# nexus-rl/dfd-starter

Hardware: AMD Instinct MI355X
Metric: env steps/sec (whole node) + sec/FD-grad-step, 4096 antithetic perturbations (higher is better)
Workload: dtype f32; 1 GPU; BASELINE config 3: HalfCheetah-shaped synthetic env (obs 17, act 6), MujocoPolicy(17,6) P=6092, 4096 antithetic perturbations per GPU (2048 directions x +/-), T=1000 fixed-length episodes, full FD step (rollout + weights + gradient + DSGD); perturbations_per_gpu=4096, envs_per_perturbation=1, global_perturbations=4096, episode_len=1000, n_params=6092, parallelism=dp1

## Files before the change

### dfd-starter_amd/csrc/fdr_common.h

```cpp
#pragma once
#include <hip/hip_runtime.h>
#include <stdint.h>

#include "../../include/fdr.h"

namespace fdr {

constexpr int kWave = 64;
constexpr int kHidden = 64;

__host__ __device__ __forceinline__ uint64_t mix64(uint64_t z) {
  z = (z ^ (z >> 30)) * 0xBF58476D1CE4E5B9ull;
  z = (z ^ (z >> 27)) * 0x94D049BB133111EBull;
  return z ^ (z >> 31);
}
__device__ __forceinline__ uint64_t hash_ctr(uint64_t key, uint64_t lane, uint64_t t, uint64_t k) {
  const uint64_t c = (lane << 32) | (t << 4) | k;
  return mix64(key + c * 0x9E3779B97F4A7C15ull);
}
constexpr uint64_t kJiggleT = (1ull << 28) - 1;

__device__ __forceinline__ float uniform24(uint64_t h) {
  return (float)(uint32_t)(h >> 40) * 0x1p-24f;
}
__device__ __forceinline__ float normal_bm(uint64_t h) {
  const float u1 = (float)((uint32_t)(h >> 40) + 1u) * 0x1p-24f;
  const float u2 = (float)((uint32_t)(h >> 16) & 0xFFFFFFu) * 0x1p-24f;
  const float r = __builtin_sqrtf(-1.38629436111989061f * __builtin_amdgcn_logf(u1));
  return r * __builtin_amdgcn_cosf(u2);
}

constexpr float kTanhScale = 2.88539008177792681f;
__device__ __forceinline__ float tanh_pre(float t) {
  const float e = __builtin_amdgcn_exp2f(t);
  return 1.0f - 2.0f * __builtin_amdgcn_rcpf(1.0f + e);
}
__device__ __forceinline__ float tanh_fast(float x) { return tanh_pre(x * kTanhScale); }
template <bool kPre>
__device__ __forceinline__ float tanh_act(float z) {
  if constexpr (kPre) return tanh_pre(z);
  else return tanh_fast(z);
}

__device__ __forceinline__ void wave_lds_sync() {
  __builtin_amdgcn_fence(__ATOMIC_RELEASE, "wavefront");
  __builtin_amdgcn_wave_barrier();
  __builtin_amdgcn_fence(__ATOMIC_ACQUIRE, "wavefront");
}

template <typename T>
__device__ __forceinline__ T wave_sum(T v) {
#pragma unroll
  for (int m = 32; m >= 1; m >>= 1) v += __shfl_xor(v, m, kWave);
  return v;
}

struct ParamSrc {
  const float* base;
  const float* eps;
  float sigma;
  int sgn;
  double n2;

  __device__ __forceinline__ float get(int64_t p) {
#pragma clang fp contract(off)
    const float t = base[p];
    const float st = sigma * eps[p];
    const double d = (double)st;
    n2 += sgn != 0 ? d * d : 0.0;
    return sgn > 0 ? t + st : (sgn < 0 ? t - st : t);
  }
  __device__ __forceinline__ float get_if(int64_t p, bool use) {
#pragma clang fp contract(off)
    const float t = base[p];
    const float st = sigma * eps[p];
    const double d = (double)st;
    n2 += (use && sgn != 0) ? d * d : 0.0;
    return sgn > 0 ? t + st : (sgn < 0 ? t - st : t);
  }
  __device__ __forceinline__ float get_nocount(int64_t p) const {
#pragma clang fp contract(off)
    const float t = base[p];
    const float st = sigma * eps[p];
    return sgn > 0 ? t + st : (sgn < 0 ? t - st : t);
  }
};

}
```

### dfd-starter_amd/csrc/fdr_rollout.hip

```cpp
#include <hip/hip_runtime.h>

#include <cfloat>
#include <cmath>
#include <cstdlib>
#include <cstring>
#include <type_traits>
#include <utility>

#include "fdr_common.h"
#include "fdr_internal.h"
#include "fdr_wave.h"

namespace fdr {

constexpr int kLanesPerBlock = 4;

#ifdef FDR_PHASE_STAMPS
__device__ unsigned long long g_phase_stamps[5];
#endif

__host__ __device__ constexpr int round4(int x) { return (x + 3) / 4 * 4; }

template <int NIN, int NA, bool DISC>
struct Layout {
// ... 636 lines not shown
          mark(2, y);
        } else {
          y = pl.layers23(h1, sc, j, mark, WIDE ? w3reg : nullptr);
        }
        int act_d = 0;
        float act_c = 0.f;
        if constexpr (DISC) {
          float p;
          p = pl.template softmax<kHead2, !kDet>(y, j);
          if constexpr (kHead2 && !kDet) {
    #pragma clang fp contract(off)
            const float tot = p + dpp_mov<kDppQuadXor1>(p);
            const float p0 = dpp_mov<0xA0>(p);
            act_d = p0 <= readlane_f(rbuf, tb) * tot ? 1 : 0;
            eacc -= (j < NA) ? disc_entropy_term(p, tot) : 0.f;
          } else {
          float pv[NA];
    #pragma unroll
          for (int i = 0; i < NA; ++i) pv[i] = readlane_f(p, i);
          float tot = pv[0];
    #pragma unroll
          for (int i = 1; i < NA; ++i) tot += pv[i];
          if constexpr (kDet) {
            float best = pv[0];
    #pragma unroll
            for (int i = 1; i < NA; ++i) {
              act_d = pv[i] > best ? i : act_d;
              best = fmaxf(best, pv[i]);
            }
          } else {
            const float target = readlane_f(rbuf, tb) * tot;
            float c = 0.f;
    #pragma unroll
            for (int i = 0; i < NA - 1; ++i) {
              c += pv[i];
              act_d += c <= target ? 1 : 0;
            }
          }
          eacc -= (j < NA) ? disc_entropy_term(p, tot) : 0.f;
          }
        } else {
          const float th = tanh_fast(y);
          const float sd = std_from_tanh(dpp_mov<kDppRowShl + NA>(th));
          eacc += __builtin_amdgcn_logf(sd);
          act_c = kDet ? th : gauss_action(th, sd, zt);
        }

        mark(3, DISC ? (float)act_d : act_c);
        if constexpr (ENV == FDR_ENV_SYNTH) {
          if constexpr (kCand) {
            s = cand[0];
    #pragma unroll
            for (int i = 1; i < NA; ++i) s = act_d == i ? cand[i] : s;
          } else {
            if constexpr (DISC) {
              pre += mrow[NX + act_d];
            } else {
              float kr[NA];
    #pragma unroll
              for (int m = 0; m < NA; ++m) kr[m] = WIDE ? kreg[m] : mrow[NX + m];
              dpp_tail<NA>(pre, act_c, kr);
            }
            s = tanh_fast(pre);
          }
          racc += (double)s;
          if constexpr (kTerm) {
            if (fabsf(readlane_f(s, a.done_dim)) > a.done_thr) {
              nsteps = t + 1;
              return;
            }
          }
        } else {
          const int prev_x = col * 7;
          const int tc = col + act_d / 3 - 1, tr = row + act_d % 3 - 1;
          if (tc >= 0 && tc < a.map_w && tr >= 0 && tr < a.map_h && a.walkable[tr * a.map_w + tc]) {
            col = tc;
            row = tr;
          }
          racc += (double)(col * 7 - prev_x);
          s = trap_obs(j, col, row);
        }
        mark(4, s);
      }
    }
  };
  if (det)
    episode(std::true_type{});
  else
    episode(std::false_type{});
#ifdef FDR_PHASE_STAMPS
  if (blockIdx.x == 0 && threadIdx.x == 0)
    for (int k = 0; k < 5; ++k) g_phase_stamps[k] = ph_acc[k];
#endif

  eacc *= 0.693147180559945309f;
  const double esum = wave_sum((j < NA) ? (double)eacc : 0.0);
  if (j == 0) {
    double r = racc;
    if (a.jiggle) r += (hash_ctr(key, ulane, kJiggleT, 15) & 1ull) ? 1e-12 : -1e-12;
    a.ret[lane] = r;
    double e = esum / (double)nsteps;
    if constexpr (!DISC) e += (double)NA * 1.4189385332046727;
    a.ent[lane] = e;
    a.steps[lane] = nsteps;
  }
  if constexpr (FEAT & 2) {
    if (j < NIN) {
      a.os_mean[(int64_t)lane * NIN + j] = os_mean;
      a.os_m2[(int64_t)lane * NIN + j] = os_m2;
    }
    if (j == 0) a.os_count[lane] = os_n;
  }
}

constexpr int kPairWaves = 2;

__device__ __forceinline__ f2 tanh2_pre(f2 t) {
  const f2 d = f2{__builtin_amdgcn_exp2f(t.x), __builtin_amdgcn_exp2f(t.y)} + f2{1.f, 1.f};
  return pk_fma(f2{-2.f, -2.f}, f2{__builtin_amdgcn_rcpf(d.x), __builtin_amdgcn_rcpf(d.y)}, f2{1.f, 1.f});
}
__device__ __forceinline__ f2 tanh2_fast(f2 x) {
  return tanh2_pre(x * f2{kTanhScale, kTanhScale});
}
constexpr float kPreScale = kTanhScale;
template <bool kPre>
__device__ __forceinline__ f2 tanh2_act(f2 z) {
  if constexpr (kPre) return tanh2_pre(z);
  else return tanh2_fast(z);
}

template <int NIN, int NA, bool DISC>
struct MlpPair {
  using L = Layout<NIN, NA, DISC>;
  static constexpr int NOUT = L::NOUT;
  static constexpr int NX = round4(NIN);
  static_assert(NX <= 32, "pair kernel: policy input wider than 32");
  static constexpr bool kBiasCol = NIN < NX;
  static constexpr bool kW1Lds = NIN > 8;
  static constexpr bool kPre = !DISC;
  static constexpr float kWS = kPre ? kTanhScale : 1.f;
  static constexpr int kW1Chunks = kW1Lds ? NX / 4 : 0;
  static constexpr int kTileF4 = (2 * kW1Chunks + 8) * kWave;
  f2 w1a[kW1Lds ? 1 : NX / 2], w1b[kW1Lds ? 1 : NX / 2];
  float b1a, b1b;
  const float4* tile;
  f2 w2[64];
  float b2a, b2b, b3;
  float a0, c0, a1a, c1a, a1b, c1b, a2a, c2a, a2b, c2b;

  __host__ __device__ static constexpr int head_unit(int rho, int k, int e) {
    return 32 * rho + 8 * (k >> 2) + 4 * e + (k & 3);
  }

  __device__ __forceinline__ void load(ParamSrc& src, int t, int tid, const float* bn_mean, const float* bn_var,
                                       float4* wave_tile) {
    const int rho = t >> 4, o = t & 15;
    const int ua = 2 * t, ub = 2 * t + 1;
    float4* my = wave_tile + tid;
    tile = my;
    auto w1v = [&](int u, int k) {
      return kWS * (k < NIN ? src.get(L::L1W + (int64_t)u * NIN + k) : (k == NIN ? src.get(L::L1B + u) : 0.f));
    };
    if constexpr (kPk) {
#pragma unroll
      for (int j = 0; j < 2 * kW1Chunks; ++j) {
        const float e0 = w1v(ua, 2 * j), f0 = w1v(ub, 2 * j), e1 = w1v(ua, 2 * j + 1), f1 = w1v(ub, 2 * j + 1);
        my[j * kWave] = float4{e0, f0, e1, f1};
      }
    } else if constexpr (kW1Lds) {
#pragma unroll
      for (int m = 0; m < kW1Chunks; ++m) {
        const float e0 = w1v(ua, 4 * m), e1 = w1v(ua, 4 * m + 1), e2 = w1v(ua, 4 * m + 2), e3 = w1v(ua, 4 * m + 3);
        my[m * kWave] = float4{e0, e1, e2, e3};
        const float f0 = w1v(ub, 4 * m), f1 = w1v(ub, 4 * m + 1), f2_ = w1v(ub, 4 * m + 2), f3 = w1v(ub, 4 * m + 3);
        my[(kW1Chunks + m) * kWave] = float4{f0, f1, f2_, f3};
      }
    } else {
#pragma unroll
      for (int p = 0; p < NX / 2; ++p) {
        const float e0 = w1v(ua, 2 * p), e1 = w1v(ua, 2 * p + 1);
        w1a[p] = f2{e0, e1};
        const float f0 = w1v(ub, 2 * p), f1 = w1v(ub, 2 * p + 1);
        w1b[p] = f2{f0, f1};
      }
    }
    b1a = kBiasCol ? 0.f : kWS * src.get(L::L1B + ua);
    b1b = kBiasCol ? 0.f : kWS * src.get(L::L1B + ub);
    __builtin_amdgcn_sched_barrier(0);
    const int q4 = t >> 2, c4 = t & 3;
#pragma unroll
    for (int p = 0; p < 4; ++p) {
      const int row0 = 8 * q4 + (c4 ^ p), row1 = row0 + 4;
#pragma unroll
      for (int k = 0; k < 16; ++k) {
        const float e0 = src.get(L::L2W + (int64_t)row0 * kHidden + 16 * c4 + k);
        const float e1 = src.get(L::L2W + (int64_t)row1 * kHidden + 16 * c4 + k);
        w2[p * 16 + k] = f2{kWS * e0, kWS * e1};
      }
#pragma unroll
      for (int k = 0; k < 16; ++k) asm volatile("" : "+v"(w2[p * 16 + k]));
      asm volatile("" : "+v"(src.n2));
      __builtin_amdgcn_sched_barrier(0);
    }
    const int u2a = 8 * q4 + c4, u2b = 8 * q4 + 4 + c4;
    b2a = kWS * src.get(L::L2B + u2a);
    b2b = kWS * src.get(L::L2B + u2b);
    {
      const bool has_o = o < NOUT;
      const int oc = has_o ? o : 0;
#pragma unroll
      for (int m = 0; m < 8; ++m) {
        float e[4];
#pragma unroll
        for (int i = 0; i < 4; ++i) {
          const int w = 4 * m + i;
          e[i] = src.get_if(L::L3W + (int64_t)oc * kHidden + head_unit(rho, w & 15, w >> 4), has_o);
        }
        my[(2 * kW1Chunks + m) * kWave] =
            has_o ? float4{kWS * e[0], kWS * e[1], kWS * e[2], kWS * e[3]} : float4{0.f, 0.f, 0.f, 0.f};
      }
      const float b3v = src.get_if(L::L3B + oc, has_o && rho == 0);
      b3 = has_o ? kWS * b3v : 0.f;
    }
    wave_lds_sync();
    a0 = c0 = a1a = c1a = a1b = c1b = a2a = c2a = a2b = c2b = 0.f;
    if constexpr (DISC) {
      const float* bm = bn_mean ? bn_mean : src.base;
      const float* bv = bn_var ? bn_var : src.base;
      auto stat = [&](int k, float& rm, float& rv) {
        const float m = bm[k], v = bv[k];
        rm = bn_mean ? m : 0.f;
        rv = bn_var ? v : 1.f;
      };
      {
        const bool in = t < NIN;
        const int tc = in ? t : 0;
        const float w = src.get_if(L::BN0W + tc, in), b = src.get_if(L::BN0B + tc, in);
        float rm, rv, a, c;
        stat(tc, rm, rv);
        bn_fold(w, b, rm, rv, a, c);
        a0 = in ? a : 0.f;
        c0 = in ? c : 0.f;
      }
      auto fold = [&](int64_t wofs, int64_t bofs, int st, int u, float& av, float& cv) {
        const float w = src.get(wofs + u), b = src.get(bofs + u);
        float rm, rv;
        stat(st + u, rm, rv);
        bn_fold(w, b, rm, rv, av, cv);
      };
      fold(L::BN1W, L::BN1B, NIN, ua, a1a, c1a);
      fold(L::BN1W, L::BN1B, NIN, ub, a1b, c1b);
      fold(L::BN2W, L::BN2B, NIN + kHidden, u2a, a2a, c2a);
      fold(L::BN2W, L::BN2B, NIN + kHidden, u2b, a2b, c2b);
    }
  }

  __device__ __forceinline__ float input_transform(float x) const {
    if constexpr (DISC) {
      return fmaf(x, a0, c0);
    } else {
      return x;
    }
  }

  __device__ __forceinline__ float act1(float z, float av, float cv) const {
    if constexpr (DISC) {
      return fmaf(fmaxf(z, 0.f), av, cv);
    } else {
      return tanh_act<kPre>(z);
    }
  }

  static constexpr bool kTail = kW1Lds && kBiasCol && NX - NIN == 3;
  static constexpr int NQ = kTail ? NX / 4 - 1 : NX / 4;
  static constexpr bool kPk = kW1Lds && kBiasCol;
  static constexpr int kPkPairs = (NIN + 2) / 2;
  struct L1Rows {
    float4 wa[kW1Lds && !kPk ? NQ : 1], wb[kW1Lds && !kPk ? NQ : 1], m[NQ];
    float2 ta, tb;
    float tm;
    float4 wp[kPk ? kPkPairs : 1];
  };
  __device__ __forceinline__ void l1_prefetch(L1Rows& r, const float* mrow) const {
    const float4* m4 = reinterpret_cast<const float4*>(mrow);
#pragma unroll
    for (int q = 0; q < NQ; ++q) {
      if constexpr (kW1Lds && !kPk) {
        r.wa[q] = tile[q * kWave];
        r.wb[q] = tile[(kW1Chunks + q) * kWave];
      }
      r.m[q] = m4[q];
    }
    if constexpr (kPk) {
#pragma unroll
      for (int j = 0; j < kPkPairs; ++j) r.wp[j] = tile[j * kWave];
      if constexpr (kTail) r.tm = mrow[4 * NQ];
    } else if constexpr (kTail) {
      r.ta = *reinterpret_cast<const float2*>(&tile[NQ * kWave]);
      r.tb = *reinterpret_cast<const float2*>(&tile[(kW1Chunks + NQ) * kWave]);
      r.tm = mrow[4 * NQ];
    }
  }

  template <bool kSameInput>
  __device__ __forceinline__ f2 layer1_env(const float* xs, const float* ss, const L1Rows& rows, float& env) const {
    const float4* x4 = reinterpret_cast<const float4*>(xs);
    const float4* s4 = reinterpret_cast<const float4*>(ss);
    return layer1_env_q<kSameInput>([&](int q) { return x4[q]; }, [&](int q) { return s4[q]; }, rows, env,
                                    kTail ? xs[4 * NQ] : 0.f, kTail ? ss[4 * NQ] : 0.f);
  }
  template <bool kSameInput, class XQ, class SQ>
  __device__ __forceinline__ f2 layer1_env_q(XQ&& xq, SQ&& sq, const L1Rows& rows, float& env, float xt,
                                             float st) const {
    f2 aa0 = {b1a, 0.f}, aa1 = {0.f, 0.f}, ab0 = {b1b, 0.f}, ab1 = {0.f, 0.f};
    f2 am0 = {0.f, 0.f}, am1 = {0.f, 0.f};
    if constexpr (kPk) {
      constexpr int NC = 2;
      f2 acc[NC];
#pragma unroll
      for (int q = 0; q < NC; ++q) acc[q] = f2{0.f, 0.f};
#pragma unroll
      for (int q = 0; q < NQ; ++q) {
        const float4 xv = xq(q), mv = rows.m[q];
        const float4 sv = kSameInput ? xv : sq(q);
#pragma unroll
        for (int i = 0; i < 4; ++i) {
          const int k = 4 * q + i;
          if (k < NIN) {
            const float4 w = rows.wp[k >> 1];
            const f2 xp = (i < 2) ? f2{xv.x, xv.y} : f2{xv.z, xv.w};
            if (kPre && k == NIN % NC) {
              const float4 wb = rows.wp[NIN >> 1];
              const f2 bias = (NIN & 1) ? f2{wb.z, wb.w} : f2{wb.x, wb.y};
              acc[k % NC] = (k & 1) ? pk_fma_bhi(f2{w.z, w.w}, xp, bias) : pk_fma_blo(f2{w.x, w.y}, xp, bias);
            } else if (k < NC)
              acc[k % NC] = (k & 1) ? pk_mul_bhi(f2{w.z, w.w}, xp) : pk_mul_blo(f2{w.x, w.y}, xp);
            else
              acc[k % NC] = (k & 1) ? pk_fma_bhi(f2{w.z, w.w}, xp, acc[k % NC]) : pk_fma_blo(f2{w.x, w.y}, xp, acc[k % NC]);
          }
        }
        am0 = pk_fma(f2{mv.x, mv.y}, f2{sv.x, sv.y}, am0);
        am1 = pk_fma(f2{mv.z, mv.w}, f2{sv.z, sv.w}, am1);
      }
      if constexpr (kTail) {
        const float4 w = rows.wp[(NIN - 1) >> 1];
        acc[(NIN - 1) % NC] = pk_fma(((NIN - 1) & 1) ? f2{w.z, w.w} : f2{w.x, w.y}, f2{xt, xt}, acc[(NIN - 1) % NC]);
        am1.x = fmaf(rows.tm, kSameInput ? xt : st, am1.x);
      }
      if constexpr (!kPre || NIN % NC >= NIN) {
        const float4 w = rows.wp[NIN >> 1];
        acc[NIN % NC] = acc[NIN % NC] + ((NIN & 1) ? f2{w.z, w.w} : f2{w.x, w.y});
      }
      const f2 h = acc[0] + acc[1];
      const f2 am = am0 + am1;
      env = am.x + am.y;
      if constexpr (DISC) {
        return f2{act1(h.x, a1a, c1a), act1(h.y, a1b, c1b)};
      } else {
        return tanh2_act<kPre>(h);
      }
    }
#pragma unroll
    for (int q = 0; q < NQ; ++q) {
      const float4 xv = xq(q), mv = rows.m[q];
      const float4 sv = kSameInput ? xv : sq(q);
      float4 wa, wb;
      if constexpr (kW1Lds) {
        wa = rows.wa[q];
        wb = rows.wb[q];
      } else {
        wa = float4{w1a[2 * q].x, w1a[2 * q].y, w1a[2 * q + 1].x, w1a[2 * q + 1].y};
        wb = float4{w1b[2 * q].x, w1b[2 * q].y, w1b[2 * q + 1].x, w1b[2 * q + 1].y};
      }
      aa0 = pk_fma(f2{wa.x, wa.y}, f2{xv.x, xv.y}, aa0);
      ab0 = pk_fma(f2{wb.x, wb.y}, f2{xv.x, xv.y}, ab0);
      am0 = pk_fma(f2{mv.x, mv.y}, f2{sv.x, sv.y}, am0);
      aa1 = pk_fma(f2{wa.z, wa.w}, f2{xv.z, xv.w}, aa1);
      ab1 = pk_fma(f2{wb.z, wb.w}, f2{xv.z, xv.w}, ab1);
      am1 = pk_fma(f2{mv.z, mv.w}, f2{sv.z, sv.w}, am1);
    }
    if constexpr (kTail) {
      aa1 = pk_fma(f2{rows.ta.x, rows.ta.y}, f2{xt, 1.f}, aa1);
      ab1 = pk_fma(f2{rows.tb.x, rows.tb.y}, f2{xt, 1.f}, ab1);
      am1.x = fmaf(rows.tm, kSameInput ? xt : st, am1.x);
    }
    const f2 am = am0 + am1, ha = aa0 + aa1, hb = ab0 + ab1;
    env = am.x + am.y;
    if constexpr (DISC) {
      return f2{act1(ha.x + ha.y, a1a, c1a), act1(hb.x + hb.y, a1b, c1b)};
    } else {
      return tanh2_act<kPre>(f2{ha.x + ha.y, hb.x + hb.y});
    }
  }

  template <class Mark>
  __device__ __forceinline__ float layers23(f2 h1, float* h1s, int t, Mark&& mark) const {
    const int c4 = t & 3;
    float x[16];
    reinterpret_cast<f2*>(h1s)[t] = h1;
    wave_lds_sync();
    lds_bcast<16>(h1s + 16 * c4, x);
    float w3[32];
#pragma unroll
    for (int m = 0; m < 8; ++m) {
      const float4 w = tile[(2 * kW1Chunks + m) * kWave];
      w3[4 * m] = w.x;
      w3[4 * m + 1] = w.y;
      w3[4 * m + 2] = w.z;
      w3[4 * m + 3] = w.w;
    }
    f2 acc[4];
#pragma unroll
    for (int p = 0; p < 4; ++p)
      acc[p] = pk_fma(w2[p * 16], f2{x[0], x[0]}, (kPre && p == 0) ? f2{b2a, b2b} : f2{0.f, 0.f});
    {
      f2 xp[8];
#pragma unroll
      for (int j = 0; j < 8; ++j) xp[j] = f2{x[2 * j], x[2 * j + 1]};
#define FDR_L2_HI "op_sel:[0,1,0] op_sel_hi:[1,1,1]"
#define FDR_L2_LO "op_sel_hi:[1,0,1]"
      asm(
          "v_pk_fma_f32 %0, %4, %64, %0 " FDR_L2_HI "\n"
          "v_pk_fma_f32 %1, %5, %64, %1 " FDR_L2_HI "\n"
          "v_pk_fma_f32 %2, %6, %64, %2 " FDR_L2_HI "\n"
          "v_pk_fma_f32 %3, %7, %64, %3 " FDR_L2_HI "\n"
          "v_pk_fma_f32 %0, %8, %65, %0 " FDR_L2_LO "\n"
          "v_pk_fma_f32 %1, %9, %65, %1 " FDR_L2_LO "\n"
          "v_pk_fma_f32 %2, %10, %65, %2 " FDR_L2_LO "\n"
          "v_pk_fma_f32 %3, %11, %65, %3 " FDR_L2_LO "\n"
          "v_pk_fma_f32 %0, %12, %65, %0 " FDR_L2_HI "\n"
          "v_pk_fma_f32 %1, %13, %65, %1 " FDR_L2_HI "\n"
          "v_pk_fma_f32 %2, %14, %65, %2 " FDR_L2_HI "\n"
          "v_pk_fma_f32 %3, %15, %65, %3 " FDR_L2_HI "\n"
          "v_pk_fma_f32 %0, %16, %66, %0 " FDR_L2_LO "\n"
          "v_pk_fma_f32 %1, %17, %66, %1 " FDR_L2_LO "\n"
          "v_pk_fma_f32 %2, %18, %66, %2 " FDR_L2_LO "\n"
          "v_pk_fma_f32 %3, %19, %66, %3 " FDR_L2_LO "\n"
          "v_pk_fma_f32 %0, %20, %66, %0 " FDR_L2_HI "\n"
          "v_pk_fma_f32 %1, %21, %66, %1 " FDR_L2_HI "\n"
          "v_pk_fma_f32 %2, %22, %66, %2 " FDR_L2_HI "\n"
          "v_pk_fma_f32 %3, %23, %66, %3 " FDR_L2_HI "\n"
          "v_pk_fma_f32 %0, %24, %67, %0 " FDR_L2_LO "\n"
          "v_pk_fma_f32 %1, %25, %67, %1 " FDR_L2_LO "\n"
          "v_pk_fma_f32 %2, %26, %67, %2 " FDR_L2_LO "\n"
          "v_pk_fma_f32 %3, %27, %67, %3 " FDR_L2_LO "\n"
          "v_pk_fma_f32 %0, %28, %67, %0 " FDR_L2_HI "\n"
          "v_pk_fma_f32 %1, %29, %67, %1 " FDR_L2_HI "\n"
          "v_pk_fma_f32 %2, %30, %67, %2 " FDR_L2_HI "\n"
          "v_pk_fma_f32 %3, %31, %67, %3 " FDR_L2_HI "\n"
          "v_pk_fma_f32 %0, %32, %68, %0 " FDR_L2_LO "\n"
          "v_pk_fma_f32 %1, %33, %68, %1 " FDR_L2_LO "\n"
          "v_pk_fma_f32 %2, %34, %68, %2 " FDR_L2_LO "\n"
          "v_pk_fma_f32 %3, %35, %68, %3 " FDR_L2_LO "\n"
          "v_pk_fma_f32 %0, %36, %68, %0 " FDR_L2_HI "\n"
          "v_pk_fma_f32 %1, %37, %68, %1 " FDR_L2_HI "\n"
          "v_pk_fma_f32 %2, %38, %68, %2 " FDR_L2_HI "\n"
          "v_pk_fma_f32 %3, %39, %68, %3 " FDR_L2_HI "\n"
          "v_pk_fma_f32 %0, %40, %69, %0 " FDR_L2_LO "\n"
          "v_pk_fma_f32 %1, %41, %69, %1 " FDR_L2_LO "\n"
          "v_pk_fma_f32 %2, %42, %69, %2 " FDR_L2_LO "\n"
          "v_pk_fma_f32 %3, %43, %69, %3 " FDR_L2_LO "\n"
          "v_pk_fma_f32 %0, %44, %69, %0 " FDR_L2_HI "\n"
          "v_pk_fma_f32 %1, %45, %69, %1 " FDR_L2_HI "\n"
          "v_pk_fma_f32 %2, %46, %69, %2 " FDR_L2_HI "\n"
          "v_pk_fma_f32 %3, %47, %69, %3 " FDR_L2_HI "\n"
          "v_pk_fma_f32 %0, %48, %70, %0 " FDR_L2_LO "\n"
          "v_pk_fma_f32 %1, %49, %70, %1 " FDR_L2_LO "\n"
          "v_pk_fma_f32 %2, %50, %70, %2 " FDR_L2_LO "\n"
          "v_pk_fma_f32 %3, %51, %70, %3 " FDR_L2_LO "\n"
          "v_pk_fma_f32 %0, %52, %70, %0 " FDR_L2_HI "\n"
          "v_pk_fma_f32 %1, %53, %70, %1 " FDR_L2_HI "\n"
          "v_pk_fma_f32 %2, %54, %70, %2 " FDR_L2_HI "\n"
          "v_pk_fma_f32 %3, %55, %70, %3 " FDR_L2_HI "\n"
          "v_pk_fma_f32 %0, %56, %71, %0 " FDR_L2_LO "\n"
          "v_pk_fma_f32 %1, %57, %71, %1 " FDR_L2_LO "\n"
          "v_pk_fma_f32 %2, %58, %71, %2 " FDR_L2_LO "\n"
          "v_pk_fma_f32 %3, %59, %71, %3 " FDR_L2_LO "\n"
          "v_pk_fma_f32 %3, %63, %71, %3 " FDR_L2_HI "\n"
          "v_pk_fma_f32 %2, %62, %71, %2 " FDR_L2_HI "\n"
          "v_pk_fma_f32 %0, %60, %71, %0 " FDR_L2_HI "\n"
          "v_pk_fma_f32 %1, %61, %71, %1 " FDR_L2_HI "\n"
          : "+v"(acc[0]), "+v"(acc[1]), "+v"(acc[2]), "+v"(acc[3])
          : "v"(w2[1]), "v"(w2[17]), "v"(w2[33]), "v"(w2[49]),
            "v"(w2[2]), "v"(w2[18]), "v"(w2[34]), "v"(w2[50]),
            "v"(w2[3]), "v"(w2[19]), "v"(w2[35]), "v"(w2[51]),
            "v"(w2[4]), "v"(w2[20]), "v"(w2[36]), "v"(w2[52]),
            "v"(w2[5]), "v"(w2[21]), "v"(w2[37]), "v"(w2[53]),
            "v"(w2[6]), "v"(w2[22]), "v"(w2[38]), "v"(w2[54]),
            "v"(w2[7]), "v"(w2[23]), "v"(w2[39]), "v"(w2[55]),
            "v"(w2[8]), "v"(w2[24]), "v"(w2[40]), "v"(w2[56]),
            "v"(w2[9]), "v"(w2[25]), "v"(w2[41]), "v"(w2[57]),
            "v"(w2[10]), "v"(w2[26]), "v"(w2[42]), "v"(w2[58]),
            "v"(w2[11]), "v"(w2[27]), "v"(w2[43]), "v"(w2[59]),
            "v"(w2[12]), "v"(w2[28]), "v"(w2[44]), "v"(w2[60]),
            "v"(w2[13]), "v"(w2[29]), "v"(w2[45]), "v"(w2[61]),
            "v"(w2[14]), "v"(w2[30]), "v"(w2[46]), "v"(w2[62]),
            "v"(w2[15]), "v"(w2[31]), "v"(w2[47]), "v"(w2[63]),
            "v"(xp[0]), "v"(xp[1]), "v"(xp[2]), "v"(xp[3]), "v"(xp[4]), "v"(xp[5]), "v"(xp[6]), "v"(xp[7]));
#undef FDR_L2_LO
#undef FDR_L2_HI
    }
    f2 zs;
    {
      float o0, o1, o2, o3;
      asm volatile(
          "v_add_f32_dpp %2, %10, %6 quad_perm:[2,3,0,1] row_mask:0xf bank_mask:0xf bound_ctrl:1\n\t"
          "v_add_f32_dpp %3, %11, %7 quad_perm:[2,3,0,1] row_mask:0xf bank_mask:0xf bound_ctrl:1\n\t"
          "v_add_f32_dpp %0, %8, %4 quad_perm:[2,3,0,1] row_mask:0xf bank_mask:0xf bound_ctrl:1\n\t"
          "v_add_f32_dpp %1, %9, %5 quad_perm:[2,3,0,1] row_mask:0xf bank_mask:0xf bound_ctrl:1\n\t"
          "v_add_f32_dpp %0, %2, %0 quad_perm:[1,0,3,2] row_mask:0xf bank_mask:0xf bound_ctrl:1\n\t"
          "v_add_f32_dpp %1, %3, %1 quad_perm:[1,0,3,2] row_mask:0xf bank_mask:0xf bound_ctrl:1\n\t"
          : "=&v"(o0), "=&v"(o1), "=&v"(o2), "=&v"(o3)
          : "v"(acc[0].x), "v"(acc[0].y), "v"(acc[1].x), "v"(acc[1].y), "v"(acc[2].x), "v"(acc[2].y), "v"(acc[3].x),
            "v"(acc[3].y));
      zs = f2{o0, o1};
    }
    const float za = kPre ? zs.x : zs.x + b2a;
    const float zb = kPre ? zs.y : zs.y + b2b;
    mark(1, za);
    float h2a, h2b;
    if constexpr (DISC) {
      h2a = fmaf(fmaxf(za, 0.f), a2a, c2a);
      h2b = fmaf(fmaxf(zb, 0.f), a2b, c2b);
    } else {
      const f2 h2 = tanh2_act<kPre>(f2{za, zb});
      h2a = h2.x;
      h2b = h2.y;
    }
    float u;
    dpp_dot_32x1(u, h2a, h2b, w3);
    float v = u;
    permlane16_swap(u, v);
    const float out = (u + v) + b3;
    mark(2, out);
    return out;
  }

  template <bool kAll = false, bool kFast = false>
  __device__ __forceinline__ float softmax(float logit, int t) const {
    const bool valid = (t & 15) < NOUT;
    const float v = valid ? logit : -FLT_MAX;
    const float mx = row16_max_n<NOUT>(v);
    if constexpr (kFast) {
      const float e = valid ? __builtin_amdgcn_exp2f((v - mx) * 1.44269504088896341f) : 0.f;
      return e * __builtin_amdgcn_rcpf(row16_sum_n<NOUT>(e));
    } else {
      const float e = valid ? expf(v - mx) : 0.f;
      return e / row16_sum_n<NOUT>(e);
    }
  }
};

struct alignas(16) PairScratch {
  float h1[2][kHidden];
  float x[2][32];
};

template <int K>
__device__ __forceinline__ float row_bcast(float v) {
  return __builtin_bit_cast(float, __builtin_amdgcn_mov_dpp(__builtin_bit_cast(int, v), 0x150 + K, 0xF, 0xF, false));
}

template <int N, int... I>
__device__ __forceinline__ void row_bcast_all(float v, float (&out)[N], std::integer_sequence<int, I...>) {
  ((out[I] = row_bcast<I>(v)), ...);
}

template <int NIN, int NA, bool DISC, int FEAT>
__global__ __launch_bounds__(64 * kPairWaves, 2) void rollout_pair_kernel(RolloutArgs a) {
  using Lane = MlpPair<NIN, NA, DISC>;
  constexpr int NX = Lane::NX;
  constexpr int NMK = NX + round4(NA);
  constexpr int MKS = NMK % 8 == 0 ? NMK + 4 : NMK;
  __shared__ float4 env4[NIN * MKS / 4];
  __shared__ float4 wtile[kPairWaves * Lane::kTileF4];
  __shared__ PairScratch scratch[kPairWaves];
  float* envMK = reinterpret_cast<float*>(env4);
  for (int e = threadIdx.x; e < NIN * MKS; e += blockDim.x) {
    const int i = e / MKS, k = e % MKS;
    envMK[e] = kPreScale * (k < NIN ? a.M[i * NIN + k] : (k >= NX && k < NX + NA ? a.K[i * NA + k - NX] : 0.f));
  }
  __syncthreads();

  const int tid = threadIdx.x & 63, wv = threadIdx.x >> 6, hh = tid >> 5, t = tid & 31;
  const int lane0 = a.lane_base + (blockIdx.x * kPairWaves + wv) * 2;
  if (lane0 >= a.n_lanes) return;
  const bool active = lane0 + hh < a.n_lanes;
  const int lane = active ? lane0 + hh : lane0;

  ParamSrc src = a.lanes.src(lane);
  const bool det = a.lanes.deterministic ? a.lanes.deterministic[lane] != 0 : false;
  Lane pl;
  pl.load(src, t, tid, a.bn_mean, a.bn_var, wtile + wv * Lane::kTileF4);
  {
    double n2 = src.n2;
#pragma unroll
    for (int m = 16; m >= 1; m >>= 1) n2 += __shfl_xor(n2, m, kWave);
    asm volatile("" : "+v"(n2));
    if (t == 0 && active && a.norm2) a.norm2[lane] = n2;
  }

  const int ji = t < NIN ? t : NIN - 1;
  constexpr bool norm_obs = (FEAT & 4) != 0;
  const float om = norm_obs ? a.obs_mean[ji] : 0.f;
  const float osd = norm_obs ? a.obs_std[ji] : 1.f;
  auto policy_input = [&](float s) {
    float x = s;
    if (norm_obs) x = fminf(fmaxf((s - om) / osd, -10.f), 10.f);
    return pl.input_transform(x);
  };
  float s = a.s0[ji];
  const int T = a.T;
  const uint64_t key = a.key;
  const uint64_t ulane = (uint64_t)(a.lanes.lane_offset + lane);
  double racc = 0.0;
  float eacc = 0.f;
  const int o = t & 15;
  constexpr int kDrawsPerStep = DISC ? 1 : NA;
  constexpr int kStepsPerBatch = 32 / kDrawsPerStep;
  constexpr bool kTerm = (FEAT & 16) != 0;
  bool alive0 = true, alive1 = true;
  int n0 = T, n1 = T;
  auto alive_me = [&]() { return hh ? alive1 : alive0; };
  float rbuf = 0.f;
  const int zbase = 4 * (32 * hh + (DISC ? 0 : (o < NA ? o : 0)));
  auto* sc = &scratch[wv];
  [[maybe_unused]] float* xs = sc->x[hh];
  float* h1s = sc->h1[hh];
  const float* mrow = envMK + ji * MKS;
  constexpr bool kSame = !DISC && !norm_obs;
  typename Lane::L1Rows l1rows;
  pl.l1_prefetch(l1rows, mrow);
  float kr[DISC ? 1 : NA];
#pragma unroll
  for (int m = 0; m < (DISC ? 1 : NA); ++m) kr[m] = mrow[NX + m];
  int tb = 0;
#ifdef FDR_PHASE_STAMPS
  uint64_t ph_acc[5] = {0, 0, 0, 0, 0};
  uint64_t ph_last = 0;
  auto mark = [&](int k, float dep) {
    uint64_t now;
    asm volatile("s_memtime %0\n\ts_waitcnt lgkmcnt(0)" : "=s"(now) : "v"(dep));
    if (k >= 0) ph_acc[k] += now - ph_last;
    ph_last = now;
  };
#else
  auto mark = [](int, float) {};
#endif
  auto draw = [&](int st) {
    const int ds = t / kDrawsPerStep, dk = t % kDrawsPerStep;
    const uint64_t hsh = hash_ctr(key, ulane, (uint64_t)(st + ds), (uint64_t)dk);
    rbuf = DISC ? uniform24(hsh) : normal_bm(hsh);
  };
  auto step = [&](int st, int tb) {
    const float zt = __builtin_bit_cast(
        float, __builtin_amdgcn_ds_bpermute(zbase + 4 * kDrawsPerStep * tb, __builtin_bit_cast(int, rbuf)));
    if constexpr (FEAT & 1) {
      if (t < NIN && active && (!kTerm || alive_me())) a.states[((int64_t)lane * T + st) * NIN + t] = s;
    }
    float pre = 0.f;
    xs[t] = t < NIN ? policy_input(s) : (t == NIN ? 1.f : 0.f);
    if constexpr (!kSame) h1s[t] = t < NIN ? s : 0.f;
    wave_lds_sync();
    const f2 h1 = pl.template layer1_env<kSame>(xs, h1s, l1rows, pre);

    mark(0, h1.x);
    const float y = pl.layers23(h1, h1s, t, mark);
    pl.l1_prefetch(l1rows, mrow);
    if constexpr (DISC) {
      const float p = det ? pl.softmax(y, t) : pl.template softmax<false, true>(y, t);
      float pv[NA];
      row_bcast_all(p, pv, std::make_integer_sequence<int, NA>{});
      float tot = 0.f;
#pragma unroll
      for (int i = 0; i < NA; ++i) tot += pv[i];
      int act_d = 0;
      if (det) {
        float best = pv[0];
#pragma unroll
        for (int i = 1; i < NA; ++i) {
          act_d = pv[i] > best ? i : act_d;
          best = fmaxf(best, pv[i]);
        }
      } else {
        const float target = zt * tot;
        float cs = 0.f;
#pragma unroll
        for (int i = 0; i < NA - 1; ++i) {
          cs += pv[i];
          act_d += cs <= target ? 1 : 0;
        }
      }
      eacc -= (o < NA && (!kTerm || alive_me())) ? disc_entropy_term(p, tot) : 0.f;
      pre += mrow[NX + act_d];
    } else {
      const float th = tanh_act<Lane::kPre>(y);
      const float sd = std_from_tanh(dpp_mov<kDppRowShl + NA>(th));
      if constexpr (kTerm)
        eacc += alive_me() ? __builtin_amdgcn_logf(sd) : 0.f;
      else
        eacc += __builtin_amdgcn_logf(sd);
      const float act_c = det ? th : gauss_action(th, sd, zt);
      mark(3, act_c);
      dpp_tail<NA>(pre, act_c, kr);
    }
    s = tanh_pre(pre);
    mark(4, s);
    if constexpr (kTerm) {
      racc += alive_me() ? (double)s : 0.0;
      const bool d0 = fabsf(readlane_f(s, a.done_dim)) > a.done_thr;
      const bool d1 = fabsf(readlane_f(s, 32 + a.done_dim)) > a.done_thr;
      if (alive0 && d0) {
        alive0 = false;
        n0 = st + 1;
      }
      if (alive1 && d1) {
        alive1 = false;
        n1 = st + 1;
      }
      return !alive0 && !alive1;
    } else {
      racc += (double)s;
      return false;
    }
  };
  if constexpr (!DISC) {
    [&] {
      int st = 0;
      for (; st + kStepsPerBatch <= T; st += kStepsPerBatch) {
        asm volatile("" ::: "memory");
        mark(-1, s);
        draw(st);
#pragma unroll
        for (int k = 0; k < kStepsPerBatch; ++k) {
          if (k) {
            asm volatile("" ::: "memory");
            mark(-1, s);
          }
          if (step(st + k, k)) return;
        }
      }
      if (st < T) {
        draw(st);
        for (int k = 0; st + k < T; ++k) {
          asm volatile("" ::: "memory");
          mark(-1, s);
          if (step(st + k, k)) return;
        }
      }
    }();
  } else {
    for (int st = 0; st < T; ++st) {
      asm volatile("" ::: "memory");
      mark(-1, s);
      if (!det && tb == 0) draw(st);
      if (step(st, tb)) break;
      tb = tb + 1 == kStepsPerBatch ? 0 : tb + 1;
    }
  }

#ifdef FDR_PHASE_STAMPS
  if (blockIdx.x == 0 && threadIdx.x == 0)
    for (int k = 0; k < 5; ++k) g_phase_stamps[k] = ph_acc[k];
#endif
  eacc *= 0.693147180559945309f;
  double esum = (t < NA) ? (double)eacc : 0.0;
#pragma unroll
  for (int m = 16; m >= 1; m >>= 1) esum += __shfl_xor(esum, m, kWave);
  if (t == 0 && active) {
    double r = racc;
    if (a.jiggle) r += (hash_ctr(key, ulane, kJiggleT, 15) & 1ull) ? 1e-12 : -1e-12;
    a.ret[lane] = r;
    const int nsteps = hh ? n1 : n0;
    double e = esum / (double)nsteps;
    if constexpr (!DISC) e += (double)NA * 1.4189385332046727;
    a.ent[lane] = e;
    a.steps[lane] = nsteps;
  }
}

#define FDR_SHAPES(X) \
  X(2, 9, true)       \
  X(4, 2, true)       \
  X(8, 4, true)       \
  X(17, 6, false)     \
  X(11, 3, false)     \
  X(8, 2, false)

int launch_policy_forward(const PolicyKey& k, const LanesArgs& lanes, int n_lanes,
                          const float* bn_mean, const float* bn_var, const float* x, float* out0,
                          float* out1, hipStream_t stream) {
  const dim3 grid((n_lanes + kLanesPerBlock - 1) / kLanesPerBlock), block(64 * kLanesPerBlock);
#define FDR_FWD(NIN, NA, DISC)                                                                  \
  if (k.n_in == NIN && k.n_act == NA && k.discrete == DISC) {                                   \
    if (Layout<NIN, NA, DISC>::P != k.n_params)                                                 \
      return set_error(FDR_ERR_INVALID, "n_params does not match the policy layout");           \
    hipLaunchKernelGGL((policy_forward_kernel<NIN, NA, DISC>), grid, block, 0, stream, lanes,   \
                       n_lanes, bn_mean, bn_var, x, out0, out1);                                \
    return check_launch("policy_forward_kernel");                                               \
  }
  FDR_SHAPES(FDR_FWD)
#undef FDR_FWD
  return set_error(FDR_ERR_UNSUPPORTED, "no compiled policy_forward for this (kind, n_in, n_act)");
}

template <int NIN, int NA, bool DISC, int ENV, bool WIDE = false>
static void launch_feat(const RolloutArgs& args, dim3 grid, dim3 block, hipStream_t stream) {
  const int feat = (args.states ? 1 : 0) | (args.os_mean ? 2 : 0) | (args.obs_mean ? 4 : 0);
#define FDR_FEAT_CASE(F) \
  case F: hipLaunchKernelGGL((rollout_kernel<NIN, NA, DISC, ENV, F, WIDE>), grid, block, 0, stream, args); break;
  const int term = (ENV == FDR_ENV_SYNTH && args.done_thr > 0.f) ? 16 : 0;
  if constexpr (!WIDE) {
    if (args.u_inject) {
      switch (feat | 8 | term) {
        FDR_FEAT_CASE(8) FDR_FEAT_CASE(9) FDR_FEAT_CASE(12) FDR_FEAT_CASE(13)
        FDR_FEAT_CASE(24) FDR_FEAT_CASE(25) FDR_FEAT_CASE(28) FDR_FEAT_CASE(29)
      }
      return;
    }
  }
  switch (feat | term) {
    FDR_FEAT_CASE(0) FDR_FEAT_CASE(1) FDR_FEAT_CASE(2) FDR_FEAT_CASE(3)
    FDR_FEAT_CASE(4) FDR_FEAT_CASE(5) FDR_FEAT_CASE(6) FDR_FEAT_CASE(7)
    FDR_FEAT_CASE(16) FDR_FEAT_CASE(17) FDR_FEAT_CASE(18) FDR_FEAT_CASE(19)
    FDR_FEAT_CASE(20) FDR_FEAT_CASE(21) FDR_FEAT_CASE(22) FDR_FEAT_CASE(23)
  }
#undef FDR_FEAT_CASE
}

template <int NIN, int NA, bool DISC>
static void launch_pair(const RolloutArgs& args, int round_lanes, hipStream_t stream) {
  const int quantum = 2 * kPairWaves;
  const int n_rounds = round_lanes > 0 ? (args.n_lanes + round_lanes - 1) / round_lanes : 1;
  const int per = ((args.n_lanes + n_rounds - 1) / n_rounds + quantum - 1) / quantum * quantum;
  const int feat = (args.states ? 1 : 0) | (args.obs_mean ? 4 : 0) | (args.done_thr > 0.f ? 16 : 0);
  RolloutArgs r = args;
  for (int base = 0; base < args.n_lanes; base += per) {
    r.lane_base = base;
    const dim3 grid((std::min(per, args.n_lanes - base) + quantum - 1) / quantum), block(64 * kPairWaves);
#define FDR_PAIR_CASE(F) \
  case F: hipLaunchKernelGGL((rollout_pair_kernel<NIN, NA, DISC, F>), grid, block, 0, stream, r); break;
    switch (feat) {
      FDR_PAIR_CASE(0) FDR_PAIR_CASE(1) FDR_PAIR_CASE(4) FDR_PAIR_CASE(5)
      FDR_PAIR_CASE(16) FDR_PAIR_CASE(17) FDR_PAIR_CASE(20) FDR_PAIR_CASE(21)
    }
#undef FDR_PAIR_CASE
  }
}

static int pair_round_lanes(const Context& ctx) { return 16 * context_cus(ctx); }

static bool use_pair_kernel(const Context& ctx, int n_lanes) {
  if (ctx.rollout_impl != FDR_ROLLOUT_AUTO) return ctx.rollout_impl == FDR_ROLLOUT_PAIR;
  return n_lanes >= 4 * 4 * context_cus(ctx);
}

static bool use_wide_kernel(const Context& ctx, int n_lanes) {
  if (ctx.rollout_impl != FDR_ROLLOUT_AUTO) return ctx.rollout_impl == FDR_ROLLOUT_WIDE;
  return n_lanes <= 2 * 4 * context_cus(ctx);
}

int launch_rollout(const Context& ctx, const PolicyKey& k, int env_kind, const RolloutArgs& args, hipStream_t stream) {
  const dim3 grid((args.n_lanes + kLanesPerBlock - 1) / kLanesPerBlock), block(64 * kLanesPerBlock);
#define FDR_ROLL(NIN, NA, DISC)                                                                 \
  if (k.n_in == NIN && k.n_act == NA && k.discrete == DISC) {                                   \
    if (Layout<NIN, NA, DISC>::P != k.n_params)                                                 \
      return set_error(FDR_ERR_INVALID, "n_params does not match the policy layout");           \
    if (env_kind == FDR_ENV_SYNTH) {                                                            \
      if (use_pair_kernel(ctx, args.n_lanes) && !args.os_mean && !args.u_inject) {                         \
        launch_pair<NIN, NA, DISC>(args, pair_round_lanes(ctx), stream);                        \
        return check_launch("rollout_pair_kernel<synth>");                                      \
      }                                                                                         \
      if (use_wide_kernel(ctx, args.n_lanes) && !args.u_inject) {                               \
        launch_feat<NIN, NA, DISC, FDR_ENV_SYNTH, true>(args, grid, block, stream);             \
        return check_launch("rollout_kernel<synth, wide>");                                     \
      }                                                                                         \
      launch_feat<NIN, NA, DISC, FDR_ENV_SYNTH>(args, grid, block, stream);                     \
      return check_launch("rollout_kernel<synth>");                                             \
    }                                                                                           \
    if constexpr (NIN == 2 && NA == 9 && DISC) {                                                \
      if (env_kind == FDR_ENV_TRAP) {                                                           \
        launch_feat<NIN, NA, DISC, FDR_ENV_TRAP>(args, grid, block, stream);                    \
        return check_launch("rollout_kernel<trap>");                                            \
      }                                                                                         \
    }                                                                                           \
    return set_error(FDR_ERR_UNSUPPORTED, "env kind not compiled for this policy shape");       \
  }
  FDR_SHAPES(FDR_ROLL)
#undef FDR_ROLL
  return set_error(FDR_ERR_UNSUPPORTED, "no compiled rollout for this (kind, n_in, n_act)");
}

}

namespace fdr {

__global__ void obs_stats_merge_kernel(const float* __restrict__ mean, const float* __restrict__ m2,
                                       const int32_t* __restrict__ count, int n, int d, float* acc_mean,
                                       float* acc_m2, int64_t* acc_count) {
#pragma clang fp contract(off)
  const int j = blockIdx.x * blockDim.x + threadIdx.x;
  int64_t c = *acc_count;
  float m = j < d ? acc_mean[j] : 0.f, v = j < d ? acc_m2[j] : 0.f;
  for (int i = 0; i < n; ++i) {
    const int64_t oc = count[i];
    if (oc == 0) continue;
    const int64_t cnt = c + oc;
    if (j < d) {
      const float om = mean[(int64_t)i * d + j], ov = m2[(int64_t)i * d + j];
      const float md = om - m;
      const float mds = md * md;
      const float cm = ((float)c * m + (float)oc * om) / (float)cnt;
      v = (v + ov) + ((mds * (float)c) * (float)oc) / (float)cnt;
      m = cm;
    }
    c = cnt;
  }
  if (j < d) {
    acc_mean[j] = m;
    acc_m2[j] = v;
  }
  __syncthreads();
  if (blockIdx.x == 0 && threadIdx.x == 0) *acc_count = c;
}

int launch_obs_stats_merge(const float* mean, const float* m2, const int32_t* count, int n, int d, float* acc_mean,
                           float* acc_m2, int64_t* acc_count, hipStream_t stream) {
  if (d > 1024) return set_error(FDR_ERR_UNSUPPORTED, "obs_dim > 1024");
  hipLaunchKernelGGL(obs_stats_merge_kernel, dim3(1), dim3(1024), 0, stream, mean, m2, count, n, d, acc_mean, acc_m2,
                     acc_count);
  return check_launch("obs_stats_merge_kernel");
}

}

#ifdef FDR_PHASE_STAMPS
extern "C" int fdr_debug_phase_read(unsigned long long* out5) {
  return hipMemcpyFromSymbol(out5, HIP_SYMBOL(fdr::g_phase_stamps), 5 * sizeof(unsigned long long)) == hipSuccess
             ? 0 : -1;
}
#endif
```

Before: 4.449 billion env steps/s.

## Pipeline next batch's Box-Muller noise draw across steps and split env dot product

Splits the counter-hash and Box-Muller normal draw into five pieces and interleaves them, one per step, into the LDS-wait window of the current batch's steps, computing the next batch's noise ahead of time. The env-measurement dot product is also split out of layer 1 so the input loads and the draw piece are scheduled before the layer-1 math behind a sched barrier. Wave priority is raised around the layer-2 output section. The aim is to hide the latency of the serial hash and transcendental chain. The cost is extra live registers and a dependence on the batch holding at least five steps; the tail path now relies on the last full batch's prefetched draw.

```diff
diff --git a/dfd-starter_amd/csrc/fdr_common.h b/dfd-starter_amd/csrc/fdr_common.h
--- a/dfd-starter_amd/csrc/fdr_common.h
+++ b/dfd-starter_amd/csrc/fdr_common.h
@@ -9,26 +9,29 @@
 constexpr int kWave = 64;
 constexpr int kHidden = 64;
 
-__host__ __device__ __forceinline__ uint64_t mix64(uint64_t z) {
-  z = (z ^ (z >> 30)) * 0xBF58476D1CE4E5B9ull;
-  z = (z ^ (z >> 27)) * 0x94D049BB133111EBull;
-  return z ^ (z >> 31);
+__host__ __device__ __forceinline__ uint64_t mix64_a(uint64_t z) { return (z ^ (z >> 30)) * 0xBF58476D1CE4E5B9ull; }
+__host__ __device__ __forceinline__ uint64_t mix64_b(uint64_t z) { return (z ^ (z >> 27)) * 0x94D049BB133111EBull; }
+__host__ __device__ __forceinline__ uint64_t mix64_c(uint64_t z) { return z ^ (z >> 31); }
+__host__ __device__ __forceinline__ uint64_t mix64(uint64_t z) { return mix64_c(mix64_b(mix64_a(z))); }
+__device__ __forceinline__ uint64_t hash_ctr_word(uint64_t key, uint64_t lane, uint64_t t, uint64_t k) {
+  const uint64_t c = (lane << 32) | (t << 4) | k;
+  return key + c * 0x9E3779B97F4A7C15ull;
 }
 __device__ __forceinline__ uint64_t hash_ctr(uint64_t key, uint64_t lane, uint64_t t, uint64_t k) {
-  const uint64_t c = (lane << 32) | (t << 4) | k;
-  return mix64(key + c * 0x9E3779B97F4A7C15ull);
+  return mix64(hash_ctr_word(key, lane, t, k));
 }
 constexpr uint64_t kJiggleT = (1ull << 28) - 1;
 
 __device__ __forceinline__ float uniform24(uint64_t h) {
   return (float)(uint32_t)(h >> 40) * 0x1p-24f;
 }
-__device__ __forceinline__ float normal_bm(uint64_t h) {
-  const float u1 = (float)((uint32_t)(h >> 40) + 1u) * 0x1p-24f;
-  const float u2 = (float)((uint32_t)(h >> 16) & 0xFFFFFFu) * 0x1p-24f;
-  const float r = __builtin_sqrtf(-1.38629436111989061f * __builtin_amdgcn_logf(u1));
-  return r * __builtin_amdgcn_cosf(u2);
+__device__ __forceinline__ float bm_u1(uint64_t h) { return (float)((uint32_t)(h >> 40) + 1u) * 0x1p-24f; }
+__device__ __forceinline__ float bm_u2(uint64_t h) { return (float)((uint32_t)(h >> 16) & 0xFFFFFFu) * 0x1p-24f; }
+__device__ __forceinline__ float bm_radius(float u1) {
+  return __builtin_sqrtf(-1.38629436111989061f * __builtin_amdgcn_logf(u1));
 }
+__device__ __forceinline__ float bm_normal(float r, float u2) { return r * __builtin_amdgcn_cosf(u2); }
+__device__ __forceinline__ float normal_bm(uint64_t h) { return bm_normal(bm_radius(bm_u1(h)), bm_u2(h)); }
 
 constexpr float kTanhScale = 2.88539008177792681f;
 __device__ __forceinline__ float tanh_pre(float t) {
diff --git a/dfd-starter_amd/csrc/fdr_rollout.hip b/dfd-starter_amd/csrc/fdr_rollout.hip
--- a/dfd-starter_amd/csrc/fdr_rollout.hip
+++ b/dfd-starter_amd/csrc/fdr_rollout.hip
@@ -962,18 +962,43 @@
     }
   }
 
-  template <bool kSameInput>
-  __device__ __forceinline__ f2 layer1_env(const float* xs, const float* ss, const L1Rows& rows, float& env) const {
+  struct SIn {
+    float4 v[NQ];
+    float t;
+  };
+  template <bool kSameInput, class Fill>
+  __device__ __forceinline__ f2 layer1_env(const float* xs, const float* ss, const L1Rows& rows, SIn& sin,
+                                           Fill&& fill) const {
     const float4* x4 = reinterpret_cast<const float4*>(xs);
     const float4* s4 = reinterpret_cast<const float4*>(ss);
-    return layer1_env_q<kSameInput>([&](int q) { return x4[q]; }, [&](int q) { return s4[q]; }, rows, env,
-                                    kTail ? xs[4 * NQ] : 0.f, kTail ? ss[4 * NQ] : 0.f);
-  }
-  template <bool kSameInput, class XQ, class SQ>
-  __device__ __forceinline__ f2 layer1_env_q(XQ&& xq, SQ&& sq, const L1Rows& rows, float& env, float xt,
-                                             float st) const {
+    SIn xin;
+#pragma unroll
+    for (int q = 0; q < NQ; ++q) {
+      xin.v[q] = x4[q];
+      sin.v[q] = kSameInput ? xin.v[q] : s4[q];
+    }
+    xin.t = kTail ? xs[4 * NQ] : 0.f;
+    sin.t = kSameInput ? xin.t : (kTail ? ss[4 * NQ] : 0.f);
+    fill();
+    __builtin_amdgcn_sched_barrier(0);
+    return layer1_q(xin, rows);
+  }
+  __device__ __forceinline__ float env_ms(const SIn& sin, const L1Rows& rows) const {
+    f2 am0 = {0.f, 0.f}, am1 = {0.f, 0.f};
+#pragma unroll
+    for (int q = 0; q < NQ; ++q) {
+      const float4 sv = sin.v[q], mv = rows.m[q];
+      am0 = pk_fma(f2{mv.x, mv.y}, f2{sv.x, sv.y}, am0);
+      am1 = pk_fma(f2{mv.z, mv.w}, f2{sv.z, sv.w}, am1);
+    }
+    if constexpr (kTail) am1.x = fmaf(rows.tm, sin.t, am1.x);
+    const f2 am = am0 + am1;
+    return am.x + am.y;
+  }
+  __device__ __forceinline__ f2 layer1_q(const SIn& xin, const L1Rows& rows) const {
+    const float xt = xin.t;
+    auto xq = [&](int q) { return xin.v[q]; };
     f2 aa0 = {b1a, 0.f}, aa1 = {0.f, 0.f}, ab0 = {b1b, 0.f}, ab1 = {0.f, 0.f};
-    f2 am0 = {0.f, 0.f}, am1 = {0.f, 0.f};
     if constexpr (kPk) {
       constexpr int NC = 2;
       f2 acc[NC];
@@ -981,8 +1006,7 @@
       for (int q = 0; q < NC; ++q) acc[q] = f2{0.f, 0.f};
 #pragma unroll
       for (int q = 0; q < NQ; ++q) {
-        const float4 xv = xq(q), mv = rows.m[q];
-        const float4 sv = kSameInput ? xv : sq(q);
+        const float4 xv = xq(q);
 #pragma unroll
         for (int i = 0; i < 4; ++i) {
           const int k = 4 * q + i;
@@ -999,21 +1023,16 @@
               acc[k % NC] = (k & 1) ? pk_fma_bhi(f2{w.z, w.w}, xp, acc[k % NC]) : pk_fma_blo(f2{w.x, w.y}, xp, acc[k % NC]);
           }
         }
-        am0 = pk_fma(f2{mv.x, mv.y}, f2{sv.x, sv.y}, am0);
-        am1 = pk_fma(f2{mv.z, mv.w}, f2{sv.z, sv.w}, am1);
       }
       if constexpr (kTail) {
         const float4 w = rows.wp[(NIN - 1) >> 1];
         acc[(NIN - 1) % NC] = pk_fma(((NIN - 1) & 1) ? f2{w.z, w.w} : f2{w.x, w.y}, f2{xt, xt}, acc[(NIN - 1) % NC]);
-        am1.x = fmaf(rows.tm, kSameInput ? xt : st, am1.x);
       }
       if constexpr (!kPre || NIN % NC >= NIN) {
         const float4 w = rows.wp[NIN >> 1];
         acc[NIN % NC] = acc[NIN % NC] + ((NIN & 1) ? f2{w.z, w.w} : f2{w.x, w.y});
       }
       const f2 h = acc[0] + acc[1];
-      const f2 am = am0 + am1;
-      env = am.x + am.y;
       if constexpr (DISC) {
         return f2{act1(h.x, a1a, c1a), act1(h.y, a1b, c1b)};
       } else {
@@ -1022,8 +1041,7 @@
     }
 #pragma unroll
     for (int q = 0; q < NQ; ++q) {
-      const float4 xv = xq(q), mv = rows.m[q];
-      const float4 sv = kSameInput ? xv : sq(q);
+      const float4 xv = xq(q);
       float4 wa, wb;
       if constexpr (kW1Lds) {
         wa = rows.wa[q];
@@ -1034,18 +1052,14 @@
       }
       aa0 = pk_fma(f2{wa.x, wa.y}, f2{xv.x, xv.y}, aa0);
       ab0 = pk_fma(f2{wb.x, wb.y}, f2{xv.x, xv.y}, ab0);
-      am0 = pk_fma(f2{mv.x, mv.y}, f2{sv.x, sv.y}, am0);
       aa1 = pk_fma(f2{wa.z, wa.w}, f2{xv.z, xv.w}, aa1);
       ab1 = pk_fma(f2{wb.z, wb.w}, f2{xv.z, xv.w}, ab1);
-      am1 = pk_fma(f2{mv.z, mv.w}, f2{sv.z, sv.w}, am1);
     }
     if constexpr (kTail) {
       aa1 = pk_fma(f2{rows.ta.x, rows.ta.y}, f2{xt, 1.f}, aa1);
       ab1 = pk_fma(f2{rows.tb.x, rows.tb.y}, f2{xt, 1.f}, ab1);
-      am1.x = fmaf(rows.tm, kSameInput ? xt : st, am1.x);
-    }
-    const f2 am = am0 + am1, ha = aa0 + aa1, hb = ab0 + ab1;
-    env = am.x + am.y;
+    }
+    const f2 ha = aa0 + aa1, hb = ab0 + ab1;
     if constexpr (DISC) {
       return f2{act1(ha.x + ha.y, a1a, c1a), act1(hb.x + hb.y, a1b, c1b)};
     } else {
@@ -1058,6 +1072,7 @@
     const int c4 = t & 3;
     float x[16];
     reinterpret_cast<f2*>(h1s)[t] = h1;
+    __builtin_amdgcn_s_setprio(0);
     wave_lds_sync();
     lds_bcast<16>(h1s + 16 * c4, x);
     float w3[32];
@@ -1161,6 +1176,7 @@
 #undef FDR_L2_HI
     }
     f2 zs;
+    __builtin_amdgcn_s_setprio(1);
     {
       float o0, o1, o2, o3;
       asm volatile(
@@ -1312,7 +1328,30 @@
     const uint64_t hsh = hash_ctr(key, ulane, (uint64_t)(st + ds), (uint64_t)dk);
     rbuf = DISC ? uniform24(hsh) : normal_bm(hsh);
   };
-  auto step = [&](int st, int tb) {
+  int dctr = ((t / kDrawsPerStep) << 4) | (t % kDrawsPerStep);
+  uint64_t dz = 0;
+  float du1 = 0.f, du2 = 0.f;
+  auto draw_part = [&](int k, int st) {
+    if (k == 0) {
+      asm volatile("" : "+v"(dctr)::"memory");
+      dz = mix64_a(key + (((uint64_t)ulane << 32) | (uint64_t)((st << 4) + dctr)) * 0x9E3779B97F4A7C15ull);
+    } else if (k == 1) {
+      asm volatile("" : "+v"(dz)::"memory");
+      dz = mix64_b(dz);
+    } else if (k == 2) {
+      asm volatile("" : "+v"(dz)::"memory");
+      const uint64_t hsh = mix64_c(dz);
+      du1 = bm_u1(hsh);
+      du2 = bm_u2(hsh);
+    } else if (k == 3) {
+      asm volatile("" : "+v"(du1)::"memory");
+      du1 = bm_radius(du1);
+    } else if (k == 4) {
+      asm volatile("" : "+v"(du1), "+v"(du2)::"memory");
+      rbuf = bm_normal(du1, du2);
+    }
+  };
+  auto step = [&](int st, int tb, auto&& fill) {
     const float zt = __builtin_bit_cast(
         float, __builtin_amdgcn_ds_bpermute(zbase + 4 * kDrawsPerStep * tb, __builtin_bit_cast(int, rbuf)));
     if constexpr (FEAT & 1) {
@@ -1322,7 +1361,9 @@
     xs[t] = t < NIN ? policy_input(s) : (t == NIN ? 1.f : 0.f);
     if constexpr (!kSame) h1s[t] = t < NIN ? s : 0.f;
     wave_lds_sync();
-    const f2 h1 = pl.template layer1_env<kSame>(xs, h1s, l1rows, pre);
+    typename Lane::SIn sin;
+    const f2 h1 = pl.template layer1_env<kSame>(xs, h1s, l1rows, sin, fill);
+    pre = pl.env_ms(sin, l1rows);
 
     mark(0, h1.x);
     const float y = pl.layers23(h1, h1s, t, mark);
@@ -1387,25 +1428,27 @@
   if constexpr (!DISC) {
     [&] {
       int st = 0;
+      draw(0);
       for (; st + kStepsPerBatch <= T; st += kStepsPerBatch) {
         asm volatile("" ::: "memory");
         mark(-1, s);
-        draw(st);
 #pragma unroll
         for (int k = 0; k < kStepsPerBatch; ++k) {
           if (k) {
             asm volatile("" ::: "memory");
             mark(-1, s);
           }
-          if (step(st + k, k)) return;
+          constexpr int kLast = kStepsPerBatch - 1;
+          static_assert(kLast >= 4, "draw_part: five parts need a batch of five steps");
+          const int part = k == kLast ? 4 : (k < 4 ? k : -1);
+          if (step(st + k, k, [&] { draw_part(part, st + kStepsPerBatch); })) return;
         }
       }
       if (st < T) {
-        draw(st);
         for (int k = 0; st + k < T; ++k) {
           asm volatile("" ::: "memory");
           mark(-1, s);
-          if (step(st + k, k)) return;
+          if (step(st + k, k, [] {})) return;
         }
       }
     }();
@@ -1414,7 +1457,7 @@
       asm volatile("" ::: "memory");
       mark(-1, s);
       if (!det && tb == 0) draw(st);
-      if (step(st, tb)) break;
+      if (step(st, tb, [] {})) break;
       tb = tb + 1 == kStepsPerBatch ? 0 : tb + 1;
     }
   }
```

Result: faster. 4.673 billion env steps/s, median of 6 (+5.0%).
